# dynatrace-oss/index4j

Measured on AMD Instinct MI355X. Metric: patterns/sec + LF-steps/sec, 1M x 8-char count() on 256 MiB log index, higher is better.
Workload: dtype int32; 1 GPU; count() batch of 1048576 random 8-char patterns per GPU on 256 MiB synthetic log text, sampleRate=32 (BASELINE.json configs[1]); 4 distinct batches rotate through the timed loop; image=expanded, text_chars=268435456, patterns_per_gpu=1048576, pattern_len=8, batches=4, count_checksum=151883111733, patterns_checked_vs_oracle=0, parallelism=dp1

## Files before the change

### index4j_amd/csrc/fmx_api.cpp

```cpp
#include "../../include/fmx.h"
#include "fmx_device.hpp"
#include "fmx_build_stage.hpp"
#include "fmx_hit_values.hpp"
#include "fmx_model.hpp"
#include "fmx_options.hpp"
#include "fmx_plan.hpp"
#include "fmx_sa_index.hpp"

#include <hip/hip_runtime.h>

#include <immintrin.h>

#include <atomic>
#include <chrono>
#include <climits>
#include <condition_variable>
#include <deque>
#include <cstdio>
#include <cstdlib>
#include <cstring>
#include <map>
#include <memory>
#include <mutex>
#include <new>
#include <string>
#include <thread>
#include <utility>
#include <vector>

namespace fmx {
#include "fmx_kernel_api.hpp"
}
namespace fmxc {
#include "fmx_kernel_api.hpp"
}
struct fmx_index;
static bool image_is_compact(const fmx_index *idx);
#define FMX_DISPATCH_FN(NAME)                                                                             \
    template <class... A>                                                                                 \
    static auto k_##NAME(const fmx_index *idx, A &&...a) {                                                \
        return image_is_compact(idx) ? fmxc::NAME(std::forward<A>(a)...) : fmx::NAME(std::forward<A>(a)...); \
    }
FMX_DISPATCH_FN(launch_suffix_level1)
FMX_DISPATCH_FN(launch_suffix_expand)
FMX_DISPATCH_FN(launch_suffix_insert)
FMX_DISPATCH_FN(launch_suffix_order1)
FMX_DISPATCH_FN(launch_win_build)
FMX_DISPATCH_FN(launch_win_other)
FMX_DISPATCH_FN(launch_win_flat)
FMX_DISPATCH_FN(launch_rows_fill)
FMX_DISPATCH_FN(launch_count_plan)
FMX_DISPATCH_FN(launch_count)
FMX_DISPATCH_FN(count_workspace_bytes)
FMX_DISPATCH_FN(launch_locate_walk)
FMX_DISPATCH_FN(walk_workspace_bytes)
FMX_DISPATCH_FN(launch_locate_all)
FMX_DISPATCH_FN(launch_extract)
FMX_DISPATCH_FN(launch_extract_packed_fill)
FMX_DISPATCH_FN(launch_extract_boundary)
FMX_DISPATCH_FN(boundary_workspace_bytes)
FMX_DISPATCH_FN(boundary_order_bytes)
FMX_DISPATCH_FN(launch_wt_rank)
FMX_DISPATCH_FN(launch_wt_inverse_select)
#undef FMX_DISPATCH_FN

struct fmx_index {
    fmx::FmModel model;
    bool has_model = false;
    bool from_stream = false;
    std::vector<uint8_t> blob;
    fmx::BlobHeader hdr;
    void *d_blob = nullptr;
    size_t d_len = 0;
    int device = -1;
    int n_cu = 256;
    bool owns_device = false;
    bool wavelet_only = false;
    bool rrr_only = false;
    std::unique_ptr<fmx::SaIndex> sa;
    double wavelet_device_seconds = 0;
    void *d_suffix_table = nullptr;
    void *d_suffix_order1 = nullptr;
    void *d_self = nullptr;
    void *d_win = nullptr;
    void *d_win_other = nullptr;
    size_t win_bytes = 0;
    uint32_t win_unclean = 0;
    void *d_rows = nullptr;
    size_t rows_bytes = 0;
    uint32_t rows_replay = 0;
    void *d_line_table = nullptr;
    size_t line_table_bytes = 0;
    int32_t line_boundary = -1;
    int32_t line_count = 0;
    int64_t n_lines = 0;
    size_t suffix_table_bytes = 0;
    uint32_t suffix_table_strings = 0;
    uint32_t suffix_table_deepest = 0;
    fmx::DevIndex dev;
    mutable std::mutex ws_mutex;
    mutable std::map<std::pair<void *, int>, std::pair<void *, size_t>> ws;
    struct Plan {
        fmx::CountPlan plan;
        const uint16_t *pat = nullptr;
        const int32_t *pat_off = nullptr;
    };
    mutable std::map<void *, Plan> plans;
    struct SideLane {
        hipStream_t s = nullptr;
        std::vector<hipEvent_t> ev;
    };
    mutable std::map<void *, SideLane> side;
};

static bool image_is_compact(const fmx_index *idx) { return idx->hdr.compact != 0; }
// ... 61 lines not shown
    d.bw_suffixes = h.bw_suffixes;
    d.bw_positions = h.bw_positions;
    d.n_positions = h.n_positions;
    d.n_c = h.n_c;
    d.map_by_symbol = h.map_by_symbol;
    d.suffix_table = nullptr;
    d.suffix_chars = 0;
    d.suffix_key_bits = fmx::fmx_code_bits_for(h.wt_sigma, fmx::options().code_bits_12.load() != 0);
    d.suffix_shift = 0;
    d.suffix_mask = 0;
    d.suffix_order1 = nullptr;
    d.win = nullptr;
    d.win_other = nullptr;
    d.win_full = nullptr;
    d.win_entry4 = 0;
    d.win_flat = 0;
    d.c_lds = nullptr;
    d.c_lut = nullptr;
    d.c_lut_shift = 0;
    d.rows = nullptr;
    d.sb_cache = nullptr;
    d.sb_cache_limit = fmx::options().sb_cache_limit;
    d.wt_size = (uint32_t)h.wt_size;
    d.self = nullptr;
}

int publish_dev_index(fmx_index *idx) {
    if (!idx->d_self) HIP_TRY(hipMalloc(&idx->d_self, sizeof(fmx::DevIndex)));
    fmx::DevIndex copy = idx->dev;
    copy.self = static_cast<const fmx::DevIndex *>(idx->d_self);
    copy.sb_cache = nullptr;
    copy.suffix_table = nullptr;
    copy.suffix_order1 = nullptr;
    copy.win = nullptr;
    copy.win_other = nullptr;
    copy.win_full = nullptr;
    copy.win_entry4 = 0;
    copy.win_flat = 0;
    copy.c_lds = nullptr;
    copy.c_lut = nullptr;
    copy.rows = nullptr;
    HIP_TRY(hipMemcpy(idx->d_self, &copy, sizeof(copy), hipMemcpyHostToDevice));
    idx->dev.self = copy.self;
    return FMX_OK;
}

int require_device(const fmx_index *idx, bool rrr_handle = false) {
    if (!idx) return fail(FMX_E_ARG, "null index");
    if (idx->sa) return fail(FMX_E_ARG, "a SuffixArray handle answers only fmx_sa_* calls");
    if (idx->rrr_only != rrr_handle)
        return fail(FMX_E_ARG, rrr_handle ? "not an RrrVector handle" : "an RrrVector handle answers only fmx_rrr_* calls");
    if (!idx->d_blob) return fail(FMX_E_NO_DEVICE, "index is not resident on a HIP device (call fmx_to_device)");
    return FMX_OK;
}

constexpr int kWsPlan = 0, kWsBoundary = 1, kWsWalk = 2, kWsSegRange = 3, kWsSegCounts = 4;
constexpr int kWsHitCounts = 5;

fmx_index::SideLane *side_lane(const fmx_index *idx, void *stream, size_t n_events) {
    std::lock_guard<std::mutex> lock(idx->ws_mutex);
    fmx_index::SideLane &l = idx->side[stream];
    if (!l.s && hipStreamCreateWithFlags(&l.s, hipStreamNonBlocking) != hipSuccess) {
        l.s = nullptr;
        (void)hipGetLastError();
        return nullptr;
    }
// ... 514 lines not shown
    if (!idx->has_model || idx->wavelet_only || idx->rrr_only)
        return fail(FMX_E_ARG, "nothing to serialize (device-attached or wavelet-only handle)");
    std::vector<uint8_t> out;
    fmx::emit_model(idx->model, framed != 0, out);
    uint8_t *p = static_cast<uint8_t *>(malloc(out.size() ? out.size() : 1));
    if (!p) return fail(FMX_E_NOMEM, "out of memory");
    memcpy(p, out.data(), out.size());
    *buf = p;
    *len = out.size();
    return FMX_OK;
    });
}

int fmx_save_key_order_modelled(const fmx_index *idx) {
    return guarded([&]() -> int {
    if (!idx) return fail(FMX_E_ARG, "null argument");
    if (!idx->has_model || idx->wavelet_only || idx->rrr_only)
        return fail(FMX_E_ARG, "nothing to serialize (device-attached or wavelet-only handle)");
    return fmx::key_order_is_modelled(idx->model) ? 1 : 0;
    });
}

void fmx_free_buffer(uint8_t *buf) { free(buf); }

static void release_device_state(fmx_index *idx) {
    if (idx->device >= 0) (void)hipSetDevice(idx->device);
    for (auto &kv : idx->ws)
        if (kv.second.first) (void)hipFree(kv.second.first);
    idx->ws.clear();
    idx->plans.clear();
    if (idx->owns_device && idx->d_blob) (void)hipFree(idx->d_blob);
    if (idx->d_suffix_table) (void)hipFree(idx->d_suffix_table);
    if (idx->d_suffix_order1) (void)hipFree(idx->d_suffix_order1);
    if (idx->d_self) (void)hipFree(idx->d_self);
    if (idx->d_win) (void)hipFree(idx->d_win);
    if (idx->d_win_other) (void)hipFree(idx->d_win_other);
    if (idx->d_rows) (void)hipFree(idx->d_rows);
    if (idx->d_line_table) (void)hipFree(idx->d_line_table);
    idx->d_line_table = nullptr;
    idx->line_table_bytes = 0;
    idx->line_boundary = -1;
    idx->line_count = 0;
    idx->n_lines = 0;
    idx->d_blob = idx->d_suffix_table = idx->d_suffix_order1 = idx->d_self = idx->d_win = idx->d_win_other = idx->d_rows = nullptr;
    idx->d_len = 0;
    idx->win_bytes = idx->suffix_table_bytes = idx->rows_bytes = 0;
    idx->rows_replay = 0;
    idx->owns_device = false;
    idx->dev = fmx::DevIndex();
    for (auto &kv : idx->side) {
        for (hipEvent_t e : kv.second.ev) (void)hipEventDestroy(e);
        if (kv.second.s) {
            (void)hipStreamSynchronize(kv.second.s);
            (void)hipStreamDestroy(kv.second.s);
        }
    }
    idx->side.clear();
    idx->device = -1;
}

void fmx_free(fmx_index *idx) {
    if (!idx) return;
    release_device_state(idx);
    delete idx;
}

int32_t fmx_input_length(const fmx_index *idx) {
    if (idx->sa) return idx->sa->length();
    return idx->has_model ? idx->model.length : idx->hdr.length;
}
int32_t fmx_alphabet_length(const fmx_index *idx) {
    return idx->has_model ? (int32_t)idx->model.map_keys.size() : idx->hdr.n_keys;
}
int32_t fmx_sample_rate(const fmx_index *idx) { return idx->has_model ? idx->model.sample_rate : idx->hdr.sample_rate; }
int32_t fmx_extract_enabled(const fmx_index *idx) {
    return idx->has_model ? (idx->model.enable_extract ? 1 : 0) : idx->hdr.enable_extract;
}
// ... 165 lines not shown
    if (bytes) *bytes = have ? (int64_t)idx->rows_bytes : 0;
    if (replay_rows) *replay_rows = have ? (int64_t)idx->rows_replay : 0;
    return FMX_OK;
    });
}

int fmx_window_cells_info(const fmx_index *idx, int64_t *bytes) {
    return guarded([&]() -> int {
    if (!idx || idx->sa) return fail(FMX_E_ARG, "not an FM-index handle");
    if (bytes) *bytes = (int64_t)idx->win_bytes;
    return FMX_OK;
    });
}

int fmx_resident_bytes(const fmx_index *idx, int64_t *image, int64_t *suffix_table, int64_t *window_directory) {
    return guarded([&]() -> int {
    if (!idx || idx->sa) return fail(FMX_E_ARG, "not an FM-index handle");
    const bool resident = idx->d_blob != nullptr;
    if (image) *image = resident ? (int64_t)idx->d_len : 0;
    if (suffix_table)
        *suffix_table = resident ? (int64_t)idx->suffix_table_bytes +
                                       (idx->d_suffix_order1 ? (int64_t)idx->hdr.wt_sigma * idx->hdr.wt_sigma * 2 * (int64_t)sizeof(float) : 0)
                                 : 0;
    if (window_directory) *window_directory = resident ? (int64_t)idx->win_bytes : 0;
    return FMX_OK;
    });
}

int fmx_device_of(const fmx_index *idx) {
    if (idx && idx->sa) return idx->sa->device;
    return (idx && idx->d_blob) ? idx->device : -1;
}

static void build_suffix_table(fmx_index *idx) {
    if (idx->d_suffix_table) {
        (void)hipFree(idx->d_suffix_table);
        idx->d_suffix_table = nullptr;
        idx->suffix_table_bytes = 0;
    }
    if (idx->d_suffix_order1) {
        (void)hipFree(idx->d_suffix_order1);
        idx->d_suffix_order1 = nullptr;
    }
    idx->suffix_table_strings = idx->suffix_table_deepest = 0;
    idx->dev.suffix_table = nullptr;
    idx->dev.suffix_order1 = nullptr;
    idx->dev.suffix_chars = 0;
    idx->dev.suffix_key_bits = fmx::fmx_code_bits_for(idx->hdr.wt_sigma, fmx::options().code_bits_12.load() != 0);
    idx->dev.suffix_shift = 0;
    idx->dev.suffix_mask = 0;
    if (idx->rrr_only || idx->wavelet_only || idx->hdr.kind != 0) return;
    const uint64_t budget = (uint64_t)fmx::options().suffix_table_mb.load() << 20;
    const int key_bits = idx->dev.suffix_key_bits;
    int max_chars = fmx::options().suffix_table_chars.load();
    if (max_chars > 64 / key_bits) max_chars = 64 / key_bits;
    if (budget == 0 || max_chars < 2 || idx->hdr.wt_sigma < 2) return;
    uint64_t limit = budget;
    if (const int frac = fmx::options().suffix_table_image_fraction.load(); frac > 0)
        limit = std::min<uint64_t>(limit, std::max<uint64_t>(idx->d_len / (uint64_t)frac, 64 << 10));
    auto slots_for = [&](uint64_t strings) {
        uint64_t slots = 1024;
        while (slots < 2 * strings) slots <<= 1;
        if (slots * sizeof(fmx::SuffixSlot) > limit && slots / 2 >= 1024 && 10 * strings <= 7 * (slots / 2)) slots >>= 1;
        return slots;
    };
    uint64_t cap64 = limit / sizeof(fmx::SuffixSlot) * 7 / 10;
    if (cap64 < 1024) cap64 = 1024;
    if (cap64 > 0x3fffffffu) cap64 = 0x3fffffffu;
    const uint32_t cap = (uint32_t)cap64;
    const uint32_t cap1 = (uint32_t)idx->hdr.wt_sigma;
    fmx::SuffixSlot *level1 = nullptr, *all = nullptr;
    uint32_t *d_count = nullptr;
    void *d_slots = nullptr;
    auto cleanup = [&]() {
        (void)hipGetLastError();
        if (level1) (void)hipFree(level1);
        if (all) (void)hipFree(all);
        if (d_count) (void)hipFree(d_count);
    };
    if (hipMalloc(reinterpret_cast<void **>(&level1), (size_t)cap1 * sizeof(fmx::SuffixSlot)) != hipSuccess ||
        hipMalloc(reinterpret_cast<void **>(&all), (size_t)cap * sizeof(fmx::SuffixSlot)) != hipSuccess ||
        hipMalloc(reinterpret_cast<void **>(&d_count), 64) != hipSuccess) {
        cleanup();
        return;
    }
    auto counted = [&](uint32_t *out) {
        return hipMemcpy(out, d_count, 4, hipMemcpyDeviceToHost) == hipSuccess;
    };
    uint32_t n_prev = 0;
    if (hipMemset(d_count, 0, 64) != hipSuccess || k_launch_suffix_level1(idx, idx->dev, level1, d_count, cap1, nullptr) != 0 ||
        !counted(&n_prev) || n_prev == 0 || n_prev > cap1) {
        cleanup();
        return;
    }
    constexpr uint64_t kLevelWorkMax = 1ull << 35;
    uint32_t begin[10] = {0};
    const fmx::SuffixSlot *prev = level1;
    uint32_t total = 0;
    int chars = 1;
    while (chars < max_chars) {
        if ((uint64_t)n_prev * (uint64_t)(idx->hdr.wt_sigma - 1) > kLevelWorkMax) break;
        const uint32_t room = cap - total;
        uint32_t n_next = 0;
        if (room == 0) break;
        if (hipMemset(d_count, 0, 64) != hipSuccess ||
            k_launch_suffix_expand(idx, idx->dev, idx->n_cu, prev, n_prev, chars, key_bits, all + total, d_count, room, nullptr) != 0 ||
            !counted(&n_next)) {
            cleanup();
            return;
        }
        if (n_next == 0 || n_next > room || slots_for((uint64_t)total + n_next) * sizeof(fmx::SuffixSlot) > limit) break;
        ++chars;
        begin[chars] = total;
        prev = all + total;
        n_prev = n_next;
        total += n_next;
        begin[chars + 1] = total;
    }
    if (chars < 2) {
        cleanup();
        return;
    }
    const uint64_t slots64 = slots_for(total);
    if (slots64 * sizeof(fmx::SuffixSlot) > std::max<uint64_t>(limit, 16 << 10) || slots64 > 0x40000000u) {
        cleanup();
        return;
    }
    const uint32_t slots = (uint32_t)slots64;
    int log2_slots = 0;
    while ((1u << log2_slots) < slots) ++log2_slots;
    fmx::DevIndex geometry = idx->dev;
    geometry.suffix_chars = chars;
    geometry.suffix_shift = (uint32_t)(64 - (log2_slots - fmx::kSuffixGroupLog2));
    geometry.suffix_mask = slots - 1;
    bool ok = hipMalloc(&d_slots, (size_t)slots * sizeof(fmx::SuffixSlot)) == hipSuccess &&
              hipMemset(d_slots, 0xff, (size_t)slots * sizeof(fmx::SuffixSlot)) == hipSuccess;
    for (int len = 2; ok && len <= chars; ++len)
        ok = k_launch_suffix_insert(idx, geometry, all + begin[len], begin[len + 1] - begin[len], len,
                                       static_cast<fmx::SuffixSlot *>(d_slots), nullptr) == 0;
    if (!ok || hipStreamSynchronize(nullptr) != hipSuccess) {
        if (d_slots) (void)hipFree(d_slots);
        cleanup();
        return;
    }
    cleanup();
    idx->d_suffix_table = d_slots;
    idx->suffix_table_bytes = (size_t)slots * sizeof(fmx::SuffixSlot);
    idx->suffix_table_strings = total;
    idx->suffix_table_deepest = begin[chars + 1] - begin[chars];
    idx->dev.suffix_table = static_cast<const fmx::SuffixSlot *>(d_slots);
    idx->dev.suffix_chars = chars;
    idx->dev.suffix_shift = geometry.suffix_shift;
    idx->dev.suffix_mask = slots - 1;
    if (key_bits == 8 && idx->hdr.wt_sigma <= fmx::kOrder1MaxSigma &&
        fmx::order1_lds_bytes(fmx::kPlanDefaultBins, idx->hdr.wt_sigma) <= fmx::kPlanCodesLdsMax) {
        void *d_o1 = nullptr;
        const size_t bytes = (size_t)idx->hdr.wt_sigma * idx->hdr.wt_sigma * 2 * sizeof(float);
        if (hipMalloc(&d_o1, bytes) == hipSuccess) {
            if (k_launch_suffix_order1(idx, idx->dev, static_cast<float *>(d_o1), nullptr) == 0 &&
                hipStreamSynchronize(nullptr) == hipSuccess) {
                idx->d_suffix_order1 = d_o1;
                idx->dev.suffix_order1 = static_cast<const float *>(d_o1);
            } else {
                (void)hipFree(d_o1);
            }
        }
    }
}

int fmx_suffix_table_info(const fmx_index *idx, int32_t *chars, int64_t *bytes) {
    return guarded([&]() -> int {
    if (!idx || idx->sa) return fail(FMX_E_ARG, "not an FM-index handle");
    if (chars) *chars = idx->dev.suffix_table ? idx->dev.suffix_chars : 0;
    if (bytes) *bytes = (int64_t)idx->suffix_table_bytes;
    return FMX_OK;
    });
}

int fmx_blob(const fmx_index *idx_c, const uint8_t **blob, size_t *len) {
    return guarded([&]() -> int {
    fmx_index *idx = const_cast<fmx_index *>(idx_c);
    if (!idx || !blob || !len) return fail(FMX_E_ARG, "null argument");
    int rc = ensure_blob(idx);
    if (rc) return rc;
// ... 2927 lines not shown
```

### index4j_amd/csrc/fmx_device.hpp

```cpp
#pragma once

#include "fmx_blob.hpp"

#include <cstdint>
#include <cstring>

#if defined(__HIPCC__)
#define FMX_HD __device__ inline __attribute__((always_inline))
#define FMX_HHD __host__ __device__ inline
#define FMX_COLD static __device__ __attribute__((noinline, unused))
#define FMX_SELF(ix) ((ix).self)
#else
#define FMX_HD inline
#define FMX_HHD inline
#define FMX_COLD inline
#define FMX_SELF(ix) (&(ix))
#endif

namespace fmx {

enum : int {
    ST_OK = 0,
    ST_NOT_ENABLED = 1,
    ST_POS_NEGATIVE = 2,
    ST_STOP_TOO_LONG = 3,
    ST_DEST_TOO_SMALL = 4,
    ST_POS_TOO_LONG = 5,
    ST_DEST_SIZE_ZERO = 6,
    ST_NO_BOUNDARY = 7,
    ST_DOES_NOT_FIT = 8,
    ST_JAVA_AIOOBE = 9
};

struct DevIndex {
    const uint8_t *base;
    const int32_t *C;
    const int32_t *look_up;
    const int16_t *char2code;
    const uint32_t *suffix_words;
    const uint32_t *pos_words;
    const SbcEntry *sbc;
    const SbDesc *sbd;
    const uint16_t *inv_global;
    RrrDesc sampled;
    int32_t length, sample_rate, enable_extract;
    int32_t wt_sigma, n_sb, bw_suffixes, bw_positions, n_positions, n_c;
    int32_t map_by_symbol;
    const struct Quad *sb_cache;
    int32_t sb_cache_limit;
    uint32_t wt_size;
    const struct SuffixSlot *suffix_table;
    int32_t suffix_chars;
    int32_t suffix_key_bits;
    uint32_t suffix_shift;
    uint32_t suffix_mask;
    const float *suffix_order1;
    const struct Quad *win;
    const uint16_t *win_other;
    const uint64_t *win_full;
    int32_t win_entry4;
    int32_t win_flat;
    const int32_t *c_lds;
    const uint16_t *c_lut;
    int32_t c_lut_shift;
    const DevIndex *self;
    const uint32_t *rows;
};
inline int fmx_code_bits_for(int32_t sigma, bool allow_12 = true) { return sigma <= 256 ? 8 : ((allow_12 && sigma <= 4096) ? 12 : 16); }
constexpr int kOrder1MaxSigma = 90;
constexpr size_t kPlanCodesLdsMax = 64 << 10;
#if defined(__HIPCC__)
__host__ __device__
#endif
constexpr size_t order1_lds_bytes(int bins, int sigma) {
    return (size_t)bins * 4 + (size_t)sigma * sigma * 8 + ((size_t)sigma + 1) * 4;
}
constexpr int kPlanDefaultBins = 1 << 12;
struct SuffixSlot {
    uint64_t key;
    uint32_t start, end;
};
constexpr uint64_t kSuffixEmpty = ~0ull;
constexpr uint64_t kSuffixHashMul = 0x9E3779B97F4A7C15ull;
constexpr int kSuffixGroupLog2 = 6;
constexpr uint32_t kSuffixGroup = 1u << kSuffixGroupLog2;

#if !defined(__HIPCC__)
inline int fmx_popc(uint32_t v) { return __builtin_popcount(v); }
inline int fmx_popcll(uint64_t v) { return __builtin_popcountll(v); }
#else
FMX_HD int fmx_popc(uint32_t v) { return __builtin_popcount(v); }
FMX_HD int fmx_popcll(uint64_t v) { return __builtin_popcountll(v); }
#endif

#if defined(__HIPCC__)
#define FMX_NO_UNROLL _Pragma("clang loop unroll(disable)")
#define FMX_OPAQUE32(v) asm volatile("" : "+v"(v))
#define FMX_OPAQUE64(v) asm volatile("" : "+v"(v))
#define FMX_PIN_QUAD(q) asm volatile("" : "+v"((q).x), "+v"((q).y), "+v"((q).z), "+v"((q).w))
#else
#define FMX_NO_UNROLL
#define FMX_OPAQUE32(v) (void)0
#define FMX_OPAQUE64(v) (void)0
#define FMX_PIN_QUAD(q) (void)0
#endif

struct Quad {
    uint32_t x, y, z, w;
};
#if defined(FMX_DIAG_LINES) && defined(__HIPCC__)
__device__ unsigned long long g_diag_base;
__device__ unsigned g_diag_lines[8][1 << 19];
#endif
FMX_HD Quad ld_quad(const void *p) {
#if defined(FMX_DIAG_LINES) && defined(__HIP_DEVICE_COMPILE__)
    {
        const unsigned long long d = (unsigned long long)p - g_diag_base;
        if (d < (1ull << 31)) {
            unsigned xcc;
            asm volatile("s_getreg_b32 %0, hwreg(HW_REG_XCC_ID)" : "=s"(xcc));
            atomicOr(&g_diag_lines[xcc & 7][d >> 12], 1u << ((d >> 7) & 31));
        }
    }
#endif
    Quad q;
    memcpy(&q, p, 16);
    return q;
}
FMX_HD uint32_t ld32u(const uint8_t *p) {
    uint32_t v;
    memcpy(&v, p, 4);
    FMX_OPAQUE32(v);
    return v;
}
// ... 1335 lines not shown

FMX_HD int32_t fm_packed_get(const uint32_t *words, int64_t index, int width) {
    return (int32_t)ld_bits(words, (uint64_t)index * (uint32_t)width, width);
}

FMX_HD void fm_seek_after(const DevIndex &ix, int32_t x, int32_t &row, int32_t &skip) {
    const int32_t s = ix.sample_rate;
    const int32_t q = x / s;
    row = fm_packed_get(ix.pos_words, (int64_t)q + 1, ix.bw_positions) + 1;
    skip = s - x % s;
    if (q == ix.n_positions - 2) skip = ix.length - x;
    if (skip > ix.length - x) skip = ix.length - x;
}

FMX_HD bool fm_suffix_extend(const DevIndex &ix, const SuffixSlot &parent, int depth, int32_t c, int key_bits, SuffixSlot &child) {
    int status = ST_OK;
    const int32_t s2 = wt_rank_folded(ix, ix.inv_global, parent.start, c, status);
    const int32_t e2 = wt_rank_folded(ix, ix.inv_global, parent.end, c, status);
    if (status != ST_OK || s2 >= e2) return false;
    child.key = parent.key | ((uint64_t)(uint32_t)c << (depth * key_bits));
    child.start = (uint32_t)s2;
    child.end = (uint32_t)e2;
    return true;
}
FMX_HD uint32_t fm_suffix_home(const DevIndex &ix, uint64_t key, int len) {
    const int top = (len - 1) * ix.suffix_key_bits;
    const uint64_t low6 = (key >> top) & (kSuffixGroup - 1);
    const uint64_t rest = key & ~((uint64_t)(kSuffixGroup - 1) << top);
    const uint64_t hash = rest * kSuffixHashMul;
    const uint32_t group = (uint32_t)(hash >> ix.suffix_shift);
    const uint32_t turn = (uint32_t)(hash >> (ix.suffix_shift - kSuffixGroupLog2)) & (kSuffixGroup - 1);
    return (group * kSuffixGroup + ((uint32_t)low6 ^ turn)) & ix.suffix_mask;
}
FMX_HD bool fm_suffix_lookup(const DevIndex &ix, uint64_t key, int len, int32_t &start, int32_t &end, int32_t &back) {
    uint32_t h = fm_suffix_home(ix, key, len);
    Quad q = ld_quad(ix.suffix_table + h);
    FMX_PIN_QUAD(q);
    uint64_t k = (uint64_t)q.x | ((uint64_t)q.y << 32);
    for (uint32_t probe = 0; k != key && k != kSuffixEmpty && probe < ix.suffix_mask / kSuffixGroup; ++probe) {
        h = (h + kSuffixGroup) & ix.suffix_mask;
        q = ld_quad(ix.suffix_table + h);
        k = (uint64_t)q.x | ((uint64_t)q.y << 32);
    }
    if (k != key) return false;
    start = (int32_t)q.z;
    end = (int32_t)q.w;
    back = len - 1;
    return true;
}
template <class CodeAt>
FMX_HD bool fm_suffix_key(const DevIndex &ix, CodeAt code_at, int len, uint64_t &key) {
    key = 0;
    bool known = true;
    for (int j = 0; j < len; ++j) {
        const uint32_t cj = (uint32_t)code_at(j);
        known = known && cj != 0;
        key |= (uint64_t)cj << (j * ix.suffix_key_bits);
    }
    return known && key != kSuffixEmpty;
}
FMX_HD int fm_suffix_len(const DevIndex &ix, int32_t m) { return m < ix.suffix_chars ? (int)m : ix.suffix_chars; }

FMX_HD int32_t fm_walk_limit(const DevIndex &ix) {
    const int64_t stretches = (int64_t)ix.sample_rate * 256;
    return (int32_t)(stretches < 4096 ? 4096 : (stretches < (int64_t)ix.length ? stretches : (int64_t)ix.length));
}

template <int kWin = kWinAsk>
FMX_HD int32_t fm_locate_hit(const DevIndex &ix, const uint16_t *inv, int32_t start, int32_t k, int32_t &distance,
                             int &status) {
    int32_t j = start + 1 + k;
    distance = 0;
    RrrView sv = rrr_view_from(Quad{ix.sampled.off_rec, ix.sampled.off_bits, (uint32_t)ix.sampled.length, (uint32_t)ix.sampled.total_ones});
    bv_bind(sv, ix, inv);
    Quad scell = {0, 0, 0, 0};
    const int32_t walk_limit = fm_walk_limit(ix);
    for (;;) {
        const int32_t p = j - 1;
        if (p < 0 || p >= sv.length) {
            status = ST_JAVA_AIOOBE;
            break;
// ... 1269 lines not shown
```

### index4j_amd/csrc/fmx_kernel_api.hpp

```cpp

int launch_suffix_level1(const fmx::DevIndex &ix, fmx::SuffixSlot *out, uint32_t *count, uint32_t cap, hipStream_t st);
int launch_suffix_expand(const fmx::DevIndex &ix, int n_cu, const fmx::SuffixSlot *in, uint32_t n_in, int depth, int key_bits,
                         fmx::SuffixSlot *out, uint32_t *count, uint32_t cap, hipStream_t st);
int launch_suffix_insert(const fmx::DevIndex &geometry, const fmx::SuffixSlot *in, uint32_t n_in, int len, fmx::SuffixSlot *slots,
                         hipStream_t st);
int launch_suffix_order1(const fmx::DevIndex &ix, float *out, hipStream_t st);
int launch_win_build(const fmx::DevIndex &ix, int n_cu, uint32_t n_win, fmx::Quad *out, uint32_t *others, hipStream_t st);
int launch_win_other(const fmx::DevIndex &ix, int n_cu, uint32_t n_win, fmx::Quad *cells, const uint32_t *first, uint16_t *entries,
                     uint32_t *open_entries, int entry4, uint64_t *full, uint32_t full_cap, hipStream_t st);
int launch_win_flat(const fmx::DevIndex &ix, int n_cu, uint32_t n_pos, uint32_t *flat, uint32_t *tail, uint64_t *full,
                    uint32_t full_cap, hipStream_t st);
int launch_rows_fill(const fmx::DevIndex &ix, int n_cu, uint32_t n_rows, uint32_t *rows, uint32_t *replay, hipStream_t st);

size_t count_workspace_bytes(const fmx::DevIndex &ix, int32_t n);
int launch_count_plan(const fmx::DevIndex &ix, int n_cu, const uint16_t *pat, const int32_t *off, int32_t n, void *workspace,
                      size_t workspace_bytes, bool head_is_zero, fmx::CountPlan *plan, hipStream_t st);
int launch_count(const fmx::DevIndex &ix, int n_cu, const uint16_t *pat, const int32_t *off, const fmx::CountPlan *plan,
                 bool plan_is_foreign, int32_t n, int32_t *counts, int32_t *lf, int32_t *status, int32_t *range, hipStream_t st);

size_t walk_workspace_bytes(const fmx::DevIndex &ix, int32_t n);
int launch_locate_walk(const fmx::DevIndex &ix, int n_cu, const int32_t *range, int32_t n, int32_t max_matches, int32_t *locs,
                       int32_t loc_cap, int32_t *found, int32_t *lf, int32_t *status, const int32_t *taken, void *workspace,
                       size_t workspace_bytes, bool head_is_zero, hipStream_t st, int64_t *set_locs, int64_t set_base);
int launch_locate_all(const fmx::DevIndex &ix, int n_cu, const int32_t *range, const int64_t *hit_off, int32_t n, int64_t first_hit,
                      int64_t n_hits, int32_t *locs, int32_t *lf, int32_t *status, hipStream_t st);

int launch_extract(const fmx::DevIndex &ix, int n_cu, const int32_t *start, const int32_t *stop, int64_t n, uint16_t *dst,
                   int32_t dst_len, int32_t offset, int32_t *out_len, int32_t *lf, int32_t *status, const int32_t *slot_found,
                   int32_t slots, int32_t fixed_len, void *order_ws, size_t order_ws_bytes, bool head_is_zero, hipStream_t st);
size_t boundary_workspace_bytes(const fmx::DevIndex &ix, int64_t n, int n_cu);
size_t boundary_order_bytes(const fmx::DevIndex &ix, int64_t n);
int launch_extract_boundary(const fmx::DevIndex &ix, int n_cu, const int32_t *from, int64_t n, uint16_t boundary, int mode,
                            uint16_t *dst, int32_t dst_len, int32_t offset, int32_t *out_len, int32_t *lf, int32_t *status,
                            int32_t *aux, void *workspace, size_t workspace_bytes, const int32_t *slot_found, int32_t slots,
                            void *order_ws, size_t order_ws_bytes, bool head_is_zero, hipStream_t st);

int launch_extract_packed_fill(const fmx::DevIndex &ix, int n_cu, const int32_t *start, const int32_t *stop, int32_t n,
                               const int64_t *text_off, const int64_t *piece_off, int64_t pieces, uint16_t *chars, int32_t *status,
                               int32_t *redo, int32_t *flags, hipStream_t st);
// ... 22 lines not shown
```

### index4j_amd/csrc/fmx_kernels.hip

```cpp
#include <atomic>
#include <cstring>

#include <hip/hip_runtime.h>

#include "fmx_device.hpp"
#include "fmx_options.hpp"
#include "fmx_plan.hpp"

#if !defined(FMX_KNS)
#define FMX_KNS fmx
#endif

namespace FMX_KNS {
using namespace fmx;
#include "fmx_kernel_api.hpp"

#if FMX_COMPACT
#define FMX_KERNEL(BLOCK) __global__ __launch_bounds__(BLOCK)
#else
#define FMX_KERNEL(BLOCK) __global__ __launch_bounds__(BLOCK) __attribute__((amdgpu_waves_per_eu(8, 8)))
#endif
#ifndef FMX_WALK_WAVES
#define FMX_WALK_WAVES 8
#endif
// ... 524 lines not shown
    if (c == 0) return;
    {
        uint64_t cc;
        memcpy(&cc, T->C + c, 8);
        start = (int32_t)(uint32_t)cc;
        end = (int32_t)(uint32_t)(cc >> 32);
    }
    const SuffixSlot *table = T->suffix_table;
    int len = 0;
    if (table) {
        const int32_t chars = T->suffix_chars;
        len = m < chars ? (int)m : (int)chars;
    }
    if (ck.n < len) len = ck.n;
    if (len >= 2) {
        const int bits = len * kCodeBits;
        const uint64_t key = bits >= 64 ? ck.lo : (ck.lo & ((1ull << bits) - 1ull));
        if ((uint32_t)(key >> (bits - kCodeBits)) != 0u && key != kSuffixEmpty) {
            const uint32_t shift = T->suffix_shift, mask = T->suffix_mask;
            const int top = bits - kCodeBits;
            const uint64_t low6 = (key >> top) & (kSuffixGroup - 1);
            const uint64_t hash = (key & ~((uint64_t)(kSuffixGroup - 1) << top)) * kSuffixHashMul;
            const uint32_t group = (uint32_t)(hash >> shift);
            const uint32_t turn = (uint32_t)(hash >> (shift - kSuffixGroupLog2)) & (kSuffixGroup - 1);
            uint32_t h = (group * kSuffixGroup + ((uint32_t)low6 ^ turn)) & mask;
            Quad q = ld_quad(table + h);
            FMX_PIN_QUAD(q);
            uint64_t k = (uint64_t)q.x | ((uint64_t)q.y << 32);
            for (uint32_t probe = 0; k != key && k != kSuffixEmpty && probe < mask / kSuffixGroup; ++probe) {
                h = (h + kSuffixGroup) & mask;
                q = ld_quad(table + h);
                k = (uint64_t)q.x | ((uint64_t)q.y << 32);
            }
            if (k == key) {
                start = (int32_t)q.z;
                end = (int32_t)q.w;
                back = len - 1;
            }
        }
        tabled = back;
    }
    while (start < end && back + 1 < m) {
        ++back;
        if (kChunks) {
            if (back - ck.base >= ck.n) ck = chunk_refill_body<kCodeBits>(T->char2code, s_map, T->pat, beg, m, back);
            c = chunk_code<kCodeBits>(ck, back - ck.base);
        } else {
            c = (int32_t)((uint32_t)(ck.lo >> (back * kCodeBits)) & code_mask);
        }
        if (c == 0) {
            start = end = 0;
            --back;
            break;
        }
        const int32_t mine = rank_lean<kMapBySymbol>(H, s_sbl, (uint32_t)(role ? end : start), (uint32_t)c);
        const int32_t other = __shfl_xor(mine, 1);
        if ((mine | other) < 0) {
            --back;
            cold = true;
            break;
        }
        start = role ? other : mine;
        end = role ? mine : other;
    }
}

template <int kBlock, int kCodeBits, bool kMapBySymbol>
// ... 129 lines not shown
    uint32_t h = fm_suffix_home(ix, me.key, len);
    for (uint32_t probe = 0; probe <= ix.suffix_mask / kSuffixGroup; ++probe, h = (h + kSuffixGroup) & ix.suffix_mask) {
        unsigned long long *key = reinterpret_cast<unsigned long long *>(&slots[h].key);
        if (atomicCAS(key, (unsigned long long)kSuffixEmpty, (unsigned long long)me.key) == (unsigned long long)kSuffixEmpty) {
            slots[h].start = me.start;
            slots[h].end = me.end;
            return;
        }
    }
}
int launch_suffix_level1(const DevIndex &ix, SuffixSlot *out, uint32_t *count, uint32_t cap, hipStream_t st) {
    DevIndex plain = ix;
    plain.sb_cache = nullptr;
    plain.suffix_table = nullptr;
    hipLaunchKernelGGL(k_suffix_level1, dim3((unsigned)((ix.wt_sigma + 255) / 256)), dim3(256), 0, st, plain, out, count, cap);
    return (int)hipGetLastError();
}
int launch_suffix_expand(const DevIndex &ix, int n_cu, const SuffixSlot *in, uint32_t n_in, int depth, int key_bits, SuffixSlot *out,
                         uint32_t *count, uint32_t cap, hipStream_t st) {
    DevIndex plain = ix;
    plain.sb_cache = nullptr;
    plain.suffix_table = nullptr;
    const uint64_t work = (uint64_t)n_in * (uint64_t)(ix.wt_sigma > 1 ? ix.wt_sigma - 1 : 1);
    uint64_t blocks = (work + 255) / 256;
    const uint64_t cap_blocks = (uint64_t)n_cu * 64;
    if (blocks > cap_blocks) blocks = cap_blocks;
    if (blocks < 1) blocks = 1;
    hipLaunchKernelGGL(k_suffix_expand, dim3((unsigned)blocks), dim3(256), 0, st, plain, in, n_in, depth, key_bits, out, count, cap);
    return (int)hipGetLastError();
}
int launch_suffix_insert(const DevIndex &geometry, const SuffixSlot *in, uint32_t n_in, int len, SuffixSlot *slots, hipStream_t st) {
    if (n_in == 0) return 0;
    hipLaunchKernelGGL(k_suffix_insert, dim3((n_in + 255) / 256), dim3(256), 0, st, geometry, in, n_in, len, slots);
    return (int)hipGetLastError();
}

__global__ __launch_bounds__(256) void k_suffix_order1(DevIndex ix, float *__restrict__ out) {
    const int sigma = ix.wt_sigma;
    const int i = (int)blockIdx.x * 256 + (int)threadIdx.x;
    if (i >= sigma * sigma) return;
    const int x = i / sigma, y = i - x * sigma;
    float f = 0.0f, p = 0.0f;
    if (x != 0 && y != 0 && x + 1 < ix.n_c) {
        int32_t s2 = 0, e2 = 0, back = 0;
        const int32_t cx = ix.C[x], nx = ix.C[x + 1] - cx;
        if (nx > 0 && fm_suffix_lookup(ix, (uint64_t)y | ((uint64_t)x << ix.suffix_key_bits), 2, s2, e2, back) && e2 > s2) {
            f = (float)(s2 - cx) / (float)nx;
            p = (float)(e2 - s2) / (float)nx;
        }
    }
    out[2 * i] = f;
    out[2 * i + 1] = p;
}
int launch_suffix_order1(const DevIndex &ix, float *out, hipStream_t st) {
    const int pairs = ix.wt_sigma * ix.wt_sigma;
    if (pairs <= 0 || ix.wt_sigma > kOrder1MaxSigma || !ix.suffix_table) return 0;
    hipLaunchKernelGGL(k_suffix_order1, dim3((pairs + 255) / 256), dim3(256), 0, st, ix, out);
    return (int)hipGetLastError();
}

__global__ __launch_bounds__(256) void k_win_build(DevIndex ix, uint32_t n_win, Quad *__restrict__ out, uint32_t *__restrict__ others) {
    for (uint64_t w = (uint64_t)blockIdx.x * 256 + threadIdx.x; w < n_win; w += (uint64_t)gridDim.x * 256) {
        uint32_t words[16];
        others[w] = win_build_cell(ix, (uint32_t)w, words);
        for (int i = 0; i < 4; ++i) out[4 * w + i] = Quad{words[4 * i], words[4 * i + 1], words[4 * i + 2], words[4 * i + 3]};
    }
// ... 1208 lines not shown
    const bool translate = recs && plan_is_foreign && pl.code_bits == 8 && plan_code_bits(ix.wt_sigma) == 8;
    const int mode = !recs ? 0 : (!plan_is_foreign ? 1 : (translate ? 2 : 3));
    DevIndex ix_launch = ix;
    if (!options().suffix_table) ix_launch.suffix_table = nullptr;
    const int bits = (mode == 1 || mode == 2) ? pl.code_bits : plan_code_bits(ix.wt_sigma);
#define FMX_COUNT_LAUNCH(BLOCK, MODE, BITS)                                                                           \
    hipLaunchKernelGGL((k_count<BLOCK, MODE, BITS>), grid__, dim3(BLOCK), (size_t)options().lds_pad_kb * 1024, st, ix_launch, pat, \
                       off, recs, n, counts, lf, status, range, pl.look_up, pl.sigma, (int)options().lf_steps_executed_only, (int)options().regroup_by_length, recs ? pl.mixed : nullptr, pl.epoch, (int)options().count_halve_uniform, (const int32_t *)nullptr, (uint32_t *)nullptr)
#define FMX_COUNT_MODE(MODE)                                                                                       \
    do {                                                                                                           \
        const int blk__ = options().block;                                                                         \
        const dim3 grid__(grid_for(2 * (int64_t)n, blk__, n_cu));                                                  \
        if (blk__ == 1024 && bits == 8)                                                                            \
            FMX_COUNT_LAUNCH(1024, MODE, 8);                                                                       \
        else if (blk__ == 1024 && bits == 12)                                                                      \
            FMX_COUNT_LAUNCH(1024, MODE, 12);                                                                      \
        else if (blk__ == 1024)                                                                                    \
            FMX_COUNT_LAUNCH(1024, MODE, 16);                                                                      \
        else if (bits == 8)                                                                                        \
            FMX_COUNT_LAUNCH(512, MODE, 8);                                                                        \
        else if (bits == 12)                                                                                       \
            FMX_COUNT_LAUNCH(512, MODE, 12);                                                                       \
        else                                                                                                       \
            FMX_COUNT_LAUNCH(512, MODE, 16);                                                                       \
    } while (0)
#if defined(FMX_DIAG_LINES)
    {
        const unsigned long long base = (unsigned long long)ix.base;
        (void)hipMemcpyToSymbolAsync(HIP_SYMBOL(g_diag_base), &base, 8, 0, hipMemcpyHostToDevice, st);
    }
#endif
#if !FMX_COMPACT
    if (mode == 1 && options().count_lean && pl.redo_list && pl.redo_count && ix.n_sb <= kSbCacheMax && ix.n_sb <= ix.sb_cache_limit &&
        (!ix_launch.suffix_table || pl.code_bits == ix.suffix_key_bits)) {
        CountLeanArgs a;
        a.hot.base = ix.base;
        a.hot.sbc = ix.sbc;
        a.hot.wt_sigma = ix.wt_sigma;
        a.hot.n_sb = ix.n_sb;
        a.hot.wt_size = ix.wt_size;
        a.hot.n = n;
        a.tile.C = ix.C;
        a.tile.suffix_table = ix_launch.suffix_table;
        a.tile.char2code = ix.char2code;
        a.tile.redo_list = pl.redo_list;
        a.tile.redo_count = pl.redo_count;
        a.tile.pat = pat;
        a.tile.pat_off = off;
        a.tile.recs = recs;
        a.tile.counts = counts;
        a.tile.lf_steps = lf;
        a.tile.status_out = status;
        a.tile.range_out = range;
        a.tile.suffix_chars = ix.suffix_chars;
        a.tile.suffix_shift = ix.suffix_shift;
        a.tile.suffix_mask = ix.suffix_mask;
        a.tile.steps_mode = (int)options().lf_steps_executed_only;
        a.tile.mixed = 0;
        a.sbd = ix.sbd;
        a.plan_mixed = pl.mixed;
        a.plan_epoch = pl.epoch;
        a.regroup = (int)options().regroup_by_length;
        a.halve_uniform = (int)options().count_halve_uniform;
        const int blk = options().block;
        const dim3 grid(grid_for(2 * (int64_t)n, blk, n_cu));
        const size_t lds = (size_t)options().lds_pad_kb * 1024;
#define FMX_LEAN_LAUNCH(BLOCK, BITS, BYSYM) hipLaunchKernelGGL((k_count_lean<BLOCK, BITS, BYSYM>), grid, dim3(BLOCK), lds, st, a)
// ... 407 lines not shown
```

Before: 8.158 billion patterns/s.

## Extend suffix table one level deeper with compact per-parent child lists

When the hashed suffix table stops growing because the next level would exceed the memory limit, the build now adds one more level as sorted per-parent child code lists with row boundaries, stored in a compact side array referenced from the parent slot's high key bits. Lookups at the deepest length find the parent slot and scan its 16-byte code groups for the child's row range. The goal is to resolve one more pattern character per lookup and so save an LF step per pattern in count(). In exchange, the lean count path is disabled whenever child lists exist, every hash probe gains a key mask, and index build gets several extra kernels and temporary buffers.

```diff
diff --git a/index4j_amd/csrc/fmx_api.cpp b/index4j_amd/csrc/fmx_api.cpp
--- a/index4j_amd/csrc/fmx_api.cpp
+++ b/index4j_amd/csrc/fmx_api.cpp
@@ -45,6 +45,11 @@
 FMX_DISPATCH_FN(launch_suffix_expand)
 FMX_DISPATCH_FN(launch_suffix_insert)
 FMX_DISPATCH_FN(launch_suffix_order1)
+FMX_DISPATCH_FN(launch_suffix_child_parents)
+FMX_DISPATCH_FN(launch_suffix_child_scan)
+FMX_DISPATCH_FN(launch_suffix_child_place)
+FMX_DISPATCH_FN(launch_suffix_child_sort)
+FMX_DISPATCH_FN(launch_suffix_child_write)
 FMX_DISPATCH_FN(launch_win_build)
 FMX_DISPATCH_FN(launch_win_other)
 FMX_DISPATCH_FN(launch_win_flat)
@@ -81,6 +86,7 @@
     double wavelet_device_seconds = 0;
     void *d_suffix_table = nullptr;
     void *d_suffix_order1 = nullptr;
+    void *d_suffix_children = nullptr;
     void *d_self = nullptr;
     void *d_win = nullptr;
     void *d_win_other = nullptr;
@@ -208,6 +214,8 @@
     copy.sb_cache = nullptr;
     copy.suffix_table = nullptr;
     copy.suffix_order1 = nullptr;
+    copy.suffix_child_rows = nullptr;
+    copy.suffix_child_codes = nullptr;
     copy.win = nullptr;
     copy.win_other = nullptr;
     copy.win_full = nullptr;
@@ -788,6 +796,7 @@
     if (idx->owns_device && idx->d_blob) (void)hipFree(idx->d_blob);
     if (idx->d_suffix_table) (void)hipFree(idx->d_suffix_table);
     if (idx->d_suffix_order1) (void)hipFree(idx->d_suffix_order1);
+    if (idx->d_suffix_children) (void)hipFree(idx->d_suffix_children);
     if (idx->d_self) (void)hipFree(idx->d_self);
     if (idx->d_win) (void)hipFree(idx->d_win);
     if (idx->d_win_other) (void)hipFree(idx->d_win_other);
@@ -798,7 +807,7 @@
     idx->line_boundary = -1;
     idx->line_count = 0;
     idx->n_lines = 0;
-    idx->d_blob = idx->d_suffix_table = idx->d_suffix_order1 = idx->d_self = idx->d_win = idx->d_win_other = idx->d_rows = nullptr;
+    idx->d_blob = idx->d_suffix_table = idx->d_suffix_order1 = idx->d_suffix_children = idx->d_self = idx->d_win = idx->d_win_other = idx->d_rows = nullptr;
     idx->d_len = 0;
     idx->win_bytes = idx->suffix_table_bytes = idx->rows_bytes = 0;
     idx->rows_replay = 0;
@@ -1030,6 +1039,69 @@
     return (idx && idx->d_blob) ? idx->device : -1;
 }
 
+constexpr uint64_t kLevelWorkMax = 1ull << 35;
+
+struct ChildLists {
+    void *d_lists = nullptr;
+    size_t codes_at = 0, bytes = 0;
+    uint32_t strings = 0;
+};
+static ChildLists grow_child_lists(const fmx_index *idx, const fmx::DevIndex &hashed, const fmx::SuffixSlot *parents, uint32_t n_parents,
+                                   int depth, fmx::SuffixSlot *table, uint32_t slots, uint64_t limit) {
+    const ChildLists none;
+    const uint64_t hashed_bytes = (uint64_t)slots * sizeof(fmx::SuffixSlot);
+    if (n_parents == 0 || limit < hashed_bytes + 4096) return none;
+    if ((uint64_t)n_parents * (uint64_t)(idx->hdr.wt_sigma - 1) > kLevelWorkMax) return none;
+    const uint32_t cap = (uint32_t)std::min<uint64_t>((limit - hashed_bytes) / 5, fmx::kSuffixChildMax);
+    std::vector<void *> temps;
+    auto temp = [&](size_t bytes) -> void * {
+        void *p = nullptr;
+        if (hipMalloc(&p, bytes) != hipSuccess) return nullptr;
+        temps.push_back(p);
+        return p;
+    };
+    auto release = [&]() {
+        (void)hipGetLastError();
+        for (void *p : temps) (void)hipFree(p);
+    };
+    auto *kids = static_cast<fmx::SuffixSlot *>(temp((size_t)cap * sizeof(fmx::SuffixSlot)));
+    auto *d_totals = static_cast<uint32_t *>(temp(64));
+    uint32_t n_kids = 0;
+    if (!kids || !d_totals || hipMemset(d_totals, 0, 64) != hipSuccess ||
+        k_launch_suffix_expand(idx, idx->dev, idx->n_cu, parents, n_parents, depth, 8, kids, d_totals, cap, nullptr) != 0 ||
+        hipMemcpy(&n_kids, d_totals, 4, hipMemcpyDeviceToHost) != hipSuccess || n_kids == 0 || n_kids > cap)
+        return release(), none;
+    auto *placed = static_cast<fmx::SuffixSlot *>(temp((size_t)n_kids * sizeof(fmx::SuffixSlot)));
+    auto *kid_slot = static_cast<uint32_t *>(temp((size_t)n_kids * 4));
+    auto *per_slot = static_cast<uint32_t *>(temp((size_t)slots * 4 * 3));
+    if (!placed || !kid_slot || !per_slot || hipMemset(per_slot, 0, (size_t)slots * 4 * 3) != hipSuccess) return release(), none;
+    uint32_t *run = per_slot + slots, *first = run + slots;
+    uint32_t totals[2] = {0, 0};
+    if (k_launch_suffix_child_parents(idx, hashed, kids, n_kids, depth + 1, table, kid_slot, per_slot, nullptr) != 0 ||
+        k_launch_suffix_child_scan(idx, per_slot, run, slots, d_totals, nullptr) != 0 ||
+        k_launch_suffix_child_place(idx, kids, n_kids, kid_slot, run, placed, nullptr) != 0 ||
+        k_launch_suffix_child_sort(idx, slots, per_slot, run, placed, first, nullptr) != 0 ||
+        k_launch_suffix_child_scan(idx, first, first, slots, d_totals + 1, nullptr) != 0 ||
+        hipMemcpy(totals, d_totals, 8, hipMemcpyDeviceToHost) != hipSuccess)
+        return release(), none;
+    if (totals[0] == 0 || totals[0] > n_kids || totals[1] <= totals[0] || totals[1] > fmx::kSuffixChildMax) return release(), none;
+    ChildLists lists;
+    lists.codes_at = (size_t)totals[1] * 4;
+    lists.bytes = (lists.codes_at + totals[1] + fmx::kSuffixChildPad + 15) & ~(size_t)15;
+    lists.strings = totals[0];
+    if (hashed_bytes + lists.bytes > limit) return release(), none;
+    if (hipMalloc(&lists.d_lists, lists.bytes) != hipSuccess) return release(), none;
+    if (hipMemset(lists.d_lists, 0, lists.bytes) != hipSuccess ||
+        k_launch_suffix_child_write(idx, slots, per_slot, run, placed, first, table, static_cast<uint32_t *>(lists.d_lists),
+                                    static_cast<uint8_t *>(lists.d_lists) + lists.codes_at, nullptr) != 0 ||
+        hipStreamSynchronize(nullptr) != hipSuccess) {
+        (void)hipFree(lists.d_lists);
+        return release(), none;
+    }
+    release();
+    return lists;
+}
+
 static void build_suffix_table(fmx_index *idx) {
     if (idx->d_suffix_table) {
         (void)hipFree(idx->d_suffix_table);
@@ -1040,6 +1112,12 @@
         (void)hipFree(idx->d_suffix_order1);
         idx->d_suffix_order1 = nullptr;
     }
+    if (idx->d_suffix_children) {
+        (void)hipFree(idx->d_suffix_children);
+        idx->d_suffix_children = nullptr;
+    }
+    idx->dev.suffix_child_rows = nullptr;
+    idx->dev.suffix_child_codes = nullptr;
     idx->suffix_table_strings = idx->suffix_table_deepest = 0;
     idx->dev.suffix_table = nullptr;
     idx->dev.suffix_order1 = nullptr;
@@ -1091,11 +1169,11 @@
         cleanup();
         return;
     }
-    constexpr uint64_t kLevelWorkMax = 1ull << 35;
     uint32_t begin[10] = {0};
     const fmx::SuffixSlot *prev = level1;
     uint32_t total = 0;
     int chars = 1;
+    bool too_large = false;
     while (chars < max_chars) {
         if ((uint64_t)n_prev * (uint64_t)(idx->hdr.wt_sigma - 1) > kLevelWorkMax) break;
         const uint32_t room = cap - total;
@@ -1107,7 +1185,10 @@
             cleanup();
             return;
         }
-        if (n_next == 0 || n_next > room || slots_for((uint64_t)total + n_next) * sizeof(fmx::SuffixSlot) > limit) break;
+        if (n_next == 0 || n_next > room || slots_for((uint64_t)total + n_next) * sizeof(fmx::SuffixSlot) > limit) {
+            too_large = n_next != 0;
+            break;
+        }
         ++chars;
         begin[chars] = total;
         prev = all + total;
@@ -1141,13 +1222,21 @@
         cleanup();
         return;
     }
+    geometry.suffix_table = static_cast<const fmx::SuffixSlot *>(d_slots);
+    ChildLists lists;
+    if (too_large && chars >= 2 && chars + 1 <= max_chars && key_bits == 8 && chars * key_bits <= fmx::kSuffixChildShift)
+        lists = grow_child_lists(idx, geometry, all + begin[chars], begin[chars + 1] - begin[chars], chars,
+                                 static_cast<fmx::SuffixSlot *>(d_slots), slots, limit);
     cleanup();
     idx->d_suffix_table = d_slots;
-    idx->suffix_table_bytes = (size_t)slots * sizeof(fmx::SuffixSlot);
-    idx->suffix_table_strings = total;
-    idx->suffix_table_deepest = begin[chars + 1] - begin[chars];
+    idx->suffix_table_bytes = (size_t)slots * sizeof(fmx::SuffixSlot) + lists.bytes;
+    idx->suffix_table_strings = total + lists.strings;
+    idx->suffix_table_deepest = lists.d_lists ? lists.strings : begin[chars + 1] - begin[chars];
+    idx->d_suffix_children = lists.d_lists;
     idx->dev.suffix_table = static_cast<const fmx::SuffixSlot *>(d_slots);
-    idx->dev.suffix_chars = chars;
+    idx->dev.suffix_chars = lists.d_lists ? chars + 1 : chars;
+    idx->dev.suffix_child_rows = static_cast<const uint32_t *>(lists.d_lists);
+    idx->dev.suffix_child_codes = lists.d_lists ? static_cast<const uint8_t *>(lists.d_lists) + lists.codes_at : nullptr;
     idx->dev.suffix_shift = geometry.suffix_shift;
     idx->dev.suffix_mask = slots - 1;
     if (key_bits == 8 && idx->hdr.wt_sigma <= fmx::kOrder1MaxSigma &&
diff --git a/index4j_amd/csrc/fmx_device.hpp b/index4j_amd/csrc/fmx_device.hpp
--- a/index4j_amd/csrc/fmx_device.hpp
+++ b/index4j_amd/csrc/fmx_device.hpp
@@ -54,6 +54,8 @@
     int32_t suffix_key_bits;
     uint32_t suffix_shift;
     uint32_t suffix_mask;
+    const uint32_t *suffix_child_rows = nullptr;
+    const uint8_t *suffix_child_codes = nullptr;
     const float *suffix_order1;
     const struct Quad *win;
     const uint16_t *win_other;
@@ -95,11 +97,13 @@
 
 #if defined(__HIPCC__)
 #define FMX_NO_UNROLL _Pragma("clang loop unroll(disable)")
+#define FMX_UNROLL _Pragma("clang loop unroll(full)")
 #define FMX_OPAQUE32(v) asm volatile("" : "+v"(v))
 #define FMX_OPAQUE64(v) asm volatile("" : "+v"(v))
 #define FMX_PIN_QUAD(q) asm volatile("" : "+v"((q).x), "+v"((q).y), "+v"((q).z), "+v"((q).w))
 #else
 #define FMX_NO_UNROLL
+#define FMX_UNROLL
 #define FMX_OPAQUE32(v) (void)0
 #define FMX_OPAQUE64(v) (void)0
 #define FMX_PIN_QUAD(q) (void)0
@@ -1501,21 +1505,89 @@
     const uint32_t turn = (uint32_t)(hash >> (ix.suffix_shift - kSuffixGroupLog2)) & (kSuffixGroup - 1);
     return (group * kSuffixGroup + ((uint32_t)low6 ^ turn)) & ix.suffix_mask;
 }
-FMX_HD bool fm_suffix_lookup(const DevIndex &ix, uint64_t key, int len, int32_t &start, int32_t &end, int32_t &back) {
+constexpr uint32_t kSuffixNoSlot = ~0u;
+constexpr int kSuffixChildShift = 40;
+constexpr uint64_t kSuffixChildKeyMask = (1ull << kSuffixChildShift) - 1ull;
+constexpr uint32_t kSuffixChildMax = 0xfffff0u;
+constexpr uint32_t kSuffixChildHole = 0x80000000u;
+constexpr uint32_t kSuffixChildPad = 32;
+FMX_HD uint32_t fm_suffix_find(const DevIndex &ix, uint64_t key, int len, Quad &q) {
+    const uint64_t keep = ix.suffix_child_rows ? kSuffixChildKeyMask : ~0ull;
     uint32_t h = fm_suffix_home(ix, key, len);
-    Quad q = ld_quad(ix.suffix_table + h);
+    q = ld_quad(ix.suffix_table + h);
     FMX_PIN_QUAD(q);
     uint64_t k = (uint64_t)q.x | ((uint64_t)q.y << 32);
-    for (uint32_t probe = 0; k != key && k != kSuffixEmpty && probe < ix.suffix_mask / kSuffixGroup; ++probe) {
+    for (uint32_t probe = 0; (k & keep) != key && k != kSuffixEmpty && probe < ix.suffix_mask / kSuffixGroup; ++probe) {
         h = (h + kSuffixGroup) & ix.suffix_mask;
         q = ld_quad(ix.suffix_table + h);
         k = (uint64_t)q.x | ((uint64_t)q.y << 32);
     }
-    if (k != key) return false;
+    return (k != kSuffixEmpty && (k & keep) == key) ? h : kSuffixNoSlot;
+}
+FMX_HD bool fm_suffix_child_lookup(const DevIndex &ix, uint64_t key, int len, int32_t &start, int32_t &end, int32_t &back) {
+    const uint32_t c = (uint32_t)key & 0xffu;
+    Quad q;
+    if (c == 0 || fm_suffix_find(ix, key >> 8, len - 1, q) == kSuffixNoSlot) return false;
+    uint32_t at = q.y >> (kSuffixChildShift - 32);
+    if (at == 0) return false;
+    --at;
+    for (int run = 0; run < 33; ++run, at += 16) {
+        const Quad w = ld_quad(ix.suffix_child_codes + at);
+        const uint32_t words[4] = {w.x, w.y, w.z, w.w};
+        int t = 16;
+        uint32_t code = 0;
+        FMX_UNROLL
+        for (int i = 15; i >= 0; --i) {
+            const uint32_t b = (words[i >> 2] >> ((i & 3) * 8)) & 0xffu;
+            if (b == 0 || b >= c) {
+                t = i;
+                code = b;
+            }
+        }
+        if (t == 16) continue;
+        if (code != c) return false;
+        const uint32_t row = ix.suffix_child_rows[at + t], next = ix.suffix_child_rows[at + t + 1];
+        if (row & kSuffixChildHole) return false;
+        start = (int32_t)row;
+        end = (int32_t)(next & ~kSuffixChildHole);
+        back = len - 1;
+        return true;
+    }
+    return false;
+}
+FMX_HD bool fm_suffix_lookup(const DevIndex &ix, uint64_t key, int len, int32_t &start, int32_t &end, int32_t &back) {
+    if (ix.suffix_child_rows && len == ix.suffix_chars) return fm_suffix_child_lookup(ix, key, len, start, end, back);
+    Quad q;
+    if (fm_suffix_find(ix, key, len, q) == kSuffixNoSlot || q.z >= q.w) return false;
     start = (int32_t)q.z;
     end = (int32_t)q.w;
     back = len - 1;
     return true;
+}
+FMX_HD void fm_suffix_child_sort(SuffixSlot *run, uint32_t n) {
+    for (uint32_t i = 1; i < n; ++i) {
+        const SuffixSlot x = run[i];
+        uint32_t j = i;
+        for (; j > 0 && (run[j - 1].key & 0xffu) > (x.key & 0xffu); --j) run[j] = run[j - 1];
+        run[j] = x;
+    }
+}
+FMX_HD uint32_t fm_suffix_child_entries(const SuffixSlot *run, uint32_t n) {
+    uint32_t entries = n + 1;
+    for (uint32_t i = 0; i + 1 < n; ++i) entries += run[i].end != run[i + 1].start;
+    return entries;
+}
+FMX_HD void fm_suffix_child_write(const SuffixSlot *run, uint32_t n, uint32_t at, uint32_t *rows, uint8_t *codes) {
+    for (uint32_t i = 0; i < n; ++i) {
+        codes[at] = (uint8_t)(run[i].key & 0xffu);
+        rows[at++] = run[i].start;
+        if (i + 1 < n && run[i].end != run[i + 1].start) {
+            codes[at] = (uint8_t)(run[i].key & 0xffu);
+            rows[at++] = run[i].end | kSuffixChildHole;
+        }
+    }
+    codes[at] = 0;
+    rows[at] = run[n - 1].end;
 }
 template <class CodeAt>
 FMX_HD bool fm_suffix_key(const DevIndex &ix, CodeAt code_at, int len, uint64_t &key) {
diff --git a/index4j_amd/csrc/fmx_kernel_api.hpp b/index4j_amd/csrc/fmx_kernel_api.hpp
--- a/index4j_amd/csrc/fmx_kernel_api.hpp
+++ b/index4j_amd/csrc/fmx_kernel_api.hpp
@@ -5,6 +5,15 @@
 int launch_suffix_insert(const fmx::DevIndex &geometry, const fmx::SuffixSlot *in, uint32_t n_in, int len, fmx::SuffixSlot *slots,
                          hipStream_t st);
 int launch_suffix_order1(const fmx::DevIndex &ix, float *out, hipStream_t st);
+int launch_suffix_child_parents(const fmx::DevIndex &hashed, const fmx::SuffixSlot *kids, uint32_t n_kids, int len,
+                                fmx::SuffixSlot *table, uint32_t *kid_slot, uint32_t *per_slot, hipStream_t st);
+int launch_suffix_child_scan(const uint32_t *in, uint32_t *out, uint32_t n, uint32_t *total, hipStream_t st);
+int launch_suffix_child_place(const fmx::SuffixSlot *kids, uint32_t n_kids, const uint32_t *kid_slot, uint32_t *cursor,
+                              fmx::SuffixSlot *placed, hipStream_t st);
+int launch_suffix_child_sort(uint32_t slots, const uint32_t *per_slot, const uint32_t *run_end, fmx::SuffixSlot *placed,
+                             uint32_t *entries, hipStream_t st);
+int launch_suffix_child_write(uint32_t slots, const uint32_t *per_slot, const uint32_t *run_end, const fmx::SuffixSlot *placed,
+                              const uint32_t *first, fmx::SuffixSlot *table, uint32_t *rows, uint8_t *codes, hipStream_t st);
 int launch_win_build(const fmx::DevIndex &ix, int n_cu, uint32_t n_win, fmx::Quad *out, uint32_t *others, hipStream_t st);
 int launch_win_other(const fmx::DevIndex &ix, int n_cu, uint32_t n_win, fmx::Quad *cells, const uint32_t *first, uint16_t *entries,
                      uint32_t *open_entries, int entry4, uint64_t *full, uint32_t full_cap, hipStream_t st);
diff --git a/index4j_amd/csrc/fmx_kernels.hip b/index4j_amd/csrc/fmx_kernels.hip
--- a/index4j_amd/csrc/fmx_kernels.hip
+++ b/index4j_amd/csrc/fmx_kernels.hip
@@ -580,7 +580,7 @@
                 q = ld_quad(table + h);
                 k = (uint64_t)q.x | ((uint64_t)q.y << 32);
             }
-            if (k == key) {
+            if (k == key && q.z < q.w) {
                 start = (int32_t)q.z;
                 end = (int32_t)q.w;
                 back = len - 1;
@@ -776,6 +776,124 @@
 int launch_suffix_insert(const DevIndex &geometry, const SuffixSlot *in, uint32_t n_in, int len, SuffixSlot *slots, hipStream_t st) {
     if (n_in == 0) return 0;
     hipLaunchKernelGGL(k_suffix_insert, dim3((n_in + 255) / 256), dim3(256), 0, st, geometry, in, n_in, len, slots);
+    return (int)hipGetLastError();
+}
+
+__global__ __launch_bounds__(256) void k_suffix_child_parents(DevIndex ix, const SuffixSlot *__restrict__ kids, uint32_t n_kids, int len,
+                                                              SuffixSlot *table, uint32_t *__restrict__ kid_slot,
+                                                              uint32_t *__restrict__ per_slot) {
+    const uint32_t i = blockIdx.x * 256 + threadIdx.x;
+    if (i >= n_kids) return;
+    Quad q;
+    const uint64_t parent = kids[i].key >> 8;
+    uint32_t h = fm_suffix_find(ix, parent, len - 1, q);
+    if (h == kSuffixNoSlot) {
+        uint32_t at = fm_suffix_home(ix, parent, len - 1);
+        for (uint32_t probe = 0; probe <= ix.suffix_mask / kSuffixGroup; ++probe, at = (at + kSuffixGroup) & ix.suffix_mask) {
+            const unsigned long long was = atomicCAS(reinterpret_cast<unsigned long long *>(&table[at].key),
+                                                     (unsigned long long)kSuffixEmpty, (unsigned long long)parent);
+            if (was == (unsigned long long)kSuffixEmpty) {
+                table[at].start = 0;
+                table[at].end = 0;
+            }
+            if (was == (unsigned long long)kSuffixEmpty || was == (unsigned long long)parent) {
+                h = at;
+                break;
+            }
+        }
+    }
+    kid_slot[i] = h;
+    if (h != kSuffixNoSlot) atomicAdd(&per_slot[h], 1u);
+}
+__global__ __launch_bounds__(1024) void k_suffix_child_scan(const uint32_t *in, uint32_t *out, uint32_t n, uint32_t *__restrict__ total) {
+    __shared__ uint32_t part[1024];
+    const uint32_t each = (n + 1023u) / 1024u;
+    const uint32_t lo = min(n, threadIdx.x * each), hi = min(n, lo + each);
+    uint32_t sum = 0;
+    for (uint32_t j = lo; j < hi; ++j) sum += in[j];
+    part[threadIdx.x] = sum;
+    __syncthreads();
+    if (threadIdx.x == 0) {
+        uint32_t run = 0;
+        for (int t = 0; t < 1024; ++t) {
+            const uint32_t v = part[t];
+            part[t] = run;
+            run += v;
+        }
+        *total = run;
+    }
+    __syncthreads();
+    uint32_t run = part[threadIdx.x];
+    for (uint32_t j = lo; j < hi; ++j) {
+        const uint32_t v = in[j];
+        out[j] = run;
+        run += v;
+    }
+}
+__global__ __launch_bounds__(256) void k_suffix_child_place(const SuffixSlot *__restrict__ kids, uint32_t n_kids,
+                                                            const uint32_t *__restrict__ kid_slot, uint32_t *__restrict__ cursor,
+                                                            SuffixSlot *__restrict__ placed) {
+    const uint32_t i = blockIdx.x * 256 + threadIdx.x;
+    if (i >= n_kids) return;
+    const uint32_t h = kid_slot[i];
+    if (h == kSuffixNoSlot) return;
+    placed[atomicAdd(&cursor[h], 1u)] = kids[i];
+}
+__global__ __launch_bounds__(256) void k_suffix_child_sort(uint32_t slots, const uint32_t *__restrict__ per_slot,
+                                                           const uint32_t *__restrict__ run_end, SuffixSlot *__restrict__ placed,
+                                                           uint32_t *__restrict__ entries) {
+    const uint32_t h = blockIdx.x * 256 + threadIdx.x;
+    if (h >= slots) return;
+    const uint32_t n = per_slot[h];
+    uint32_t e = 0;
+    if (n != 0) {
+        SuffixSlot *run = placed + (run_end[h] - n);
+        fm_suffix_child_sort(run, n);
+        e = fm_suffix_child_entries(run, n);
+    }
+    entries[h] = e;
+}
+__global__ __launch_bounds__(256) void k_suffix_child_write(uint32_t slots, const uint32_t *__restrict__ per_slot,
+                                                            const uint32_t *__restrict__ run_end, const SuffixSlot *__restrict__ placed,
+                                                            const uint32_t *__restrict__ first, SuffixSlot *__restrict__ table,
+                                                            uint32_t *__restrict__ rows, uint8_t *__restrict__ codes) {
+    const uint32_t h = blockIdx.x * 256 + threadIdx.x;
+    if (h >= slots) return;
+    const uint32_t n = per_slot[h];
+    if (n == 0) return;
+    fm_suffix_child_write(placed + (run_end[h] - n), n, first[h], rows, codes);
+    table[h].key |= (uint64_t)(first[h] + 1u) << kSuffixChildShift;
+}
+int launch_suffix_child_parents(const DevIndex &hashed, const SuffixSlot *kids, uint32_t n_kids, int len, SuffixSlot *table,
+                                uint32_t *kid_slot, uint32_t *per_slot, hipStream_t st) {
+    if (n_kids == 0) return 0;
+    DevIndex plain = hashed;
+    plain.sb_cache = nullptr;
+    plain.suffix_child_rows = nullptr;
+    plain.suffix_child_codes = nullptr;
+    hipLaunchKernelGGL(k_suffix_child_parents, dim3((n_kids + 255) / 256), dim3(256), 0, st, plain, kids, n_kids, len, table, kid_slot,
+                       per_slot);
+    return (int)hipGetLastError();
+}
+int launch_suffix_child_scan(const uint32_t *in, uint32_t *out, uint32_t n, uint32_t *total, hipStream_t st) {
+    hipLaunchKernelGGL(k_suffix_child_scan, dim3(1), dim3(1024), 0, st, in, out, n, total);
+    return (int)hipGetLastError();
+}
+int launch_suffix_child_place(const SuffixSlot *kids, uint32_t n_kids, const uint32_t *kid_slot, uint32_t *cursor, SuffixSlot *placed,
+                              hipStream_t st) {
+    if (n_kids == 0) return 0;
+    hipLaunchKernelGGL(k_suffix_child_place, dim3((n_kids + 255) / 256), dim3(256), 0, st, kids, n_kids, kid_slot, cursor, placed);
+    return (int)hipGetLastError();
+}
+int launch_suffix_child_sort(uint32_t slots, const uint32_t *per_slot, const uint32_t *run_end, SuffixSlot *placed, uint32_t *entries,
+                             hipStream_t st) {
+    hipLaunchKernelGGL(k_suffix_child_sort, dim3((slots + 255) / 256), dim3(256), 0, st, slots, per_slot, run_end, placed, entries);
+    return (int)hipGetLastError();
+}
+int launch_suffix_child_write(uint32_t slots, const uint32_t *per_slot, const uint32_t *run_end, const SuffixSlot *placed,
+                              const uint32_t *first, SuffixSlot *table, uint32_t *rows, uint8_t *codes, hipStream_t st) {
+    hipLaunchKernelGGL(k_suffix_child_write, dim3((slots + 255) / 256), dim3(256), 0, st, slots, per_slot, run_end, placed, first, table,
+                       rows, codes);
     return (int)hipGetLastError();
 }
 
@@ -2050,7 +2168,7 @@
 #endif
 #if !FMX_COMPACT
     if (mode == 1 && options().count_lean && pl.redo_list && pl.redo_count && ix.n_sb <= kSbCacheMax && ix.n_sb <= ix.sb_cache_limit &&
-        (!ix_launch.suffix_table || pl.code_bits == ix.suffix_key_bits)) {
+        (!ix_launch.suffix_table || (pl.code_bits == ix.suffix_key_bits && !ix.suffix_child_rows))) {
         CountLeanArgs a;
         a.hot.base = ix.base;
         a.hot.sbc = ix.sbc;
```

Result: faster. 8.882 billion patterns/s, median of 6 (+8.9%).
